# sokunmin/Improved-Body-Parts

Measured on AMD Instinct MI355X. Metric: end-to-end images/sec at 512×512, higher is better.
Workload: dtype f16; 1 GPU; configs[2]+forward: 512x512, flip=on, host->HBM ingest + 4-stage IMHN forward (fp16) + full HIP pafprocess (NMS + limb line-integral + assembly); launch=hipGraph replay, parallelism=image-sharded x1

## Files before the change

improved-body-parts_amd/csrc/posepaf_conv_own.hip:

```cpp
#include <hip/hip_fp16.h>
#include <hip/hip_runtime.h>

#include <atomic>
#include <cstdint>
#include <cstdlib>
#include <type_traits>

#include "../../include/posepaf.h"

namespace {

typedef _Float16 half8_t __attribute__((ext_vector_type(8)));
typedef _Float16 half4_t __attribute__((ext_vector_type(4)));
typedef float float4_t __attribute__((ext_vector_type(4)));

constexpr int BM = 256;
constexpr int NTHREADS = 512;
constexpr int SUB = 1024;

struct ConvParams {
    const _Float16 *x, *w, *bias, *extra, *extra2;
    _Float16 *y, *y2;
    const void *zero;
    int N, H, W, C, K, R, pad, dil, Ho, Wo;
// ... 319 lines not shown
        for (int i = 0; i < PT; i++) xf[i] = *reinterpret_cast<const half8_t *>(sa + (wm * PT + i) * SUB + fragoff);
        const int inflight = np - 1 - ph < 3 ? np - 1 - ph : 3;
        if (inflight == 3) wait_vmcnt<2 * NL>();
        else if (inflight == 2) wait_vmcnt<NL>();
        else if (inflight == 1) wait_vmcnt<0>();
        asm volatile("s_waitcnt lgkmcnt(0)" ::: "memory");
        __builtin_amdgcn_s_barrier();
        __builtin_amdgcn_s_setprio(1);
#pragma unroll
        for (int i = 0; i < PT; i++)
#pragma unroll
            for (int j = 0; j < CT; j++) acc[i][j] = __builtin_amdgcn_mfma_f32_16x16x32_f16(wf[j], xf[i], acc[i][j], 0, 0, 0);
        __builtin_amdgcn_s_setprio(0);
        __builtin_amdgcn_s_barrier();
    }
    if (grp == 0) __builtin_amdgcn_s_barrier();

    epilogue_store<PT, CT>(acc, p, lane, n0 + wn * 64, [&](int i) -> long {
        const long m = m0 + wm * PM + i * 16 + (lane & 15);
        if (m >= p.M) return -1;
        if (!p.up_out) return m;
        const int n = (int)(m / HoWo), rem = (int)(m - (long)n * HoWo);
        const int oy_ = rem / p.Wo, ox_ = rem - oy_ * p.Wo;
        return ((long)n * (2 * p.Ho) + 2 * oy_ + p.py) * (2 * p.Wo) + 2 * ox_ + p.px;
    }, true);
}

constexpr int TP = 512;
constexpr int HALO_RES_SUMS = 2048;
constexpr int HALO_DBG_BITS = HALO_RES_SUMS - 1;

struct HaloParams {
    int TW, TH, lgTW;
    int tiles_x, tiles;
    int HWp, nhalo, npieces;
    int gimg, hrows;
    int tps;
};

__device__ unsigned long long g_conv_clk[8 * 512];

template <int BN, int MASK, int LGTW, int PH = -1, int D = 1>
__global__ __launch_bounds__(NTHREADS) void k_conv3x3_halo(const ConvParams p, const HaloParams hp) {
    constexpr int NT = PH < 0 ? 9 : 4;
    static_assert(D == 1 || PH < 0, "the collapsed upsample form has no dilation");
    constexpr int TW = 1 << LGTW, HWp = TW + 2 * D, TH = TP / TW;
    constexpr int dbg = MASK & HALO_DBG_BITS;
    constexpr int WN = BN / 64;
    constexpr int WM = 8 / WN;
    constexpr int PM = TP / WM;
    constexpr int PT = PM / 16;
    constexpr int CT = 4;
    constexpr int WB = BN * 32 * 2;
    constexpr int KEEP = 3;
    constexpr int NW = 6;
    constexpr int AHEAD = NW - 1;
    constexpr int HP = 56;
#ifdef PP_HALO_NPW7
    constexpr int NPW = 7;
#else
    constexpr int NPW = (LGTW == 7 || D > 1) ? 7 : 6;
#endif
    static_assert(BN == 128, "one weight sub-tile per wave and phase");
    extern __shared__ __align__(16) unsigned char smem[];
    constexpr int halo_bytes = HP * SUB;
    unsigned char *s_halo = smem;
    unsigned char *s_w = smem + 2 * halo_bytes;

    const int lane = threadIdx.x & 63;
    const int wave = __builtin_amdgcn_readfirstlane(threadIdx.x >> 6);
    const int wm = wave / WN, wn = wave % WN;
    const int nct = (p.K + BN - 1) / BN;
    const int ptiles = (p.N / hp.gimg) * hp.tiles, per_xcd = (ptiles + 7) >> 3;
    const int total_ids = 8 * per_xcd * nct;
    const char *wb = reinterpret_cast<const char *>(p.w);
    int n_img = 0, ty0 = 0, tx0 = 0, n0 = 0, t_idx = 0;
    const char *xb = nullptr;
    int hsrc[7];
    const bool p4 = __builtin_amdgcn_readfirstlane(32 + wave < hp.npieces);
    const bool p5 = __builtin_amdgcn_readfirstlane(40 + wave < hp.npieces);
    const bool p6 = __builtin_amdgcn_readfirstlane(48 + wave < hp.npieces);
    unsigned woff = 0;
    int bx_lo = 0, bx_hi = 0, bw_lo = 0, bw_hi = 0, nx = 0, bw_n = 0;
    auto rsrc_of = [&](int lo, int hi, int nbytes) {
        void *base = reinterpret_cast<void *>(((unsigned long long)(unsigned)hi << 32) | (unsigned)lo);
        return __builtin_amdgcn_make_buffer_rsrc(base, 0, nbytes, 0x00020000);
    };
    auto decode = [&](int id) -> bool {
        const int xcd = id & 7, q = id >> 3;
        const int ptile = xcd * per_xcd + q / nct, ctile = q - (q / nct) * nct;
        if (q / nct >= per_xcd || ptile >= ptiles) return false;
        n_img = (ptile / hp.tiles) * hp.gimg;
        const int tile = ptile - (ptile / hp.tiles) * hp.tiles;
        t_idx = tile;
        if (D == 1) ty0 = (tile / hp.tiles_x) * TH;
        else {
            const int trow_ = tile / hp.tiles_x, cls = trow_ / hp.tps;
            ty0 = cls + (trow_ - cls * hp.tps) * TH * D;
        }
        tx0 = (tile - (tile / hp.tiles_x) * hp.tiles_x) * TW;
        n0 = ctile * BN;
        const int sw_ = p.up ? p.W >> 1 : p.W;
        const int ldx = p.ldx ? p.ldx : p.C;
        xb = reinterpret_cast<const char *>(p.x) + (long)n_img * (p.up ? p.H >> 1 : p.H) * sw_ * ldx * 2;
        int ln = lane;
        asm volatile("" : "+v"(ln));
#pragma unroll
        for (int t = 0; t < NPW; t++) {
            const int piece = t * 8 + wave;
            const int phys = piece * SUB + ln * 16;
            const int logical = phys ^ (((phys >> 8) & 1) << 5);
            const int hpix = logical >> 6, chunk = (logical >> 4) & 3;
            const int hy = hpix / HWp, hx = hpix - hy * HWp;
            const int gi = D == 1 ? hy / hp.hrows : 0;
            const int iy = D == 1 ? ty0 - 1 + (hy - gi * hp.hrows) : ty0 + (hy - 1) * D, ix = tx0 - D + hx;
            const bool ok = hpix < hp.nhalo && (unsigned)iy < (unsigned)p.H && (unsigned)ix < (unsigned)p.W;
            hsrc[t] = ok ? (((gi * (p.H >> p.up) + (iy >> p.up)) * sw_ + (ix >> p.up)) * ldx * 2 + chunk * 16)
                         : (int)0x80000000;
        }
        const int b = ln * 16;
        const int bs = b ^ (((b >> 9) & 1) << 5);
        woff = (unsigned)((bs >> 6) * (NT * p.C * 2) + (bs & 63));
        const unsigned long long ax = reinterpret_cast<unsigned long long>(xb);
        const unsigned long long aw = reinterpret_cast<unsigned long long>(wb) + (unsigned long long)((long)(n0 + wave * 16) * ((long)NT * p.C * 2));
        bx_lo = __builtin_amdgcn_readfirstlane((int)(unsigned)ax), bx_hi = __builtin_amdgcn_readfirstlane((int)(unsigned)(ax >> 32));
        bw_lo = __builtin_amdgcn_readfirstlane((int)(unsigned)aw), bw_hi = __builtin_amdgcn_readfirstlane((int)(unsigned)(aw >> 32));
        nx = __builtin_amdgcn_readfirstlane(hp.gimg * (p.up ? p.H >> 1 : p.H) * sw_ * ldx * 2);
        bw_n = __builtin_amdgcn_readfirstlane(n0 + wave * 16 < p.K ? 16 * NT * p.C * 2 : 0);
        return true;
    };
    auto next_tile = [&](int id) -> int {
        while (id < total_ids && !decode(id)) id += gridDim.x;
        return id;
    };

    const int ncb = p.C / 32;
    const int np = ncb * NT;
    int st_cb = 0, st_tap = 0;
    int st_slot = 0;
    int slot_cur = 0;
    auto stage_w = [&]() {
        lds_dma16_buf(rsrc_of(bw_lo, bw_hi, bw_n), woff, (unsigned)((st_tap * p.C + st_cb * 32) * 2), s_w + st_slot * WB + wave * SUB);
        if (++st_slot == NW) st_slot = 0;
        if (++st_tap == NT) {
            st_tap = 0;
            ++st_cb;
        }
    };
    auto stage_halo = [&](int t, int cb, int buf) {
        lds_dma16_buf(rsrc_of(bx_lo, bx_hi, nx), (unsigned)hsrc[t], (unsigned)(cb * 64), s_halo + buf * halo_bytes + (t * 8 + wave) * SUB);
    };

    const int wfrag = (lane & 15) * 64 + (((lane >> 4) * 16) ^ (((lane & 15) >> 3) << 5));
    const int rows_before = (wm * PM) >> LGTW;
    const int hb0 = ((rows_before + (hp.gimg > 1 ? 2 * (rows_before / p.H) : 0)) * HWp + ((wm * PM) & (TW - 1)) + (lane & 15)) * 64 +
                    (lane >> 4) * 16;
    const unsigned lds_halo = (unsigned)(uintptr_t)(__attribute__((address_space(3))) unsigned char *)s_halo;
    const unsigned lds_w = (unsigned)(uintptr_t)(__attribute__((address_space(3))) unsigned char *)s_w + wn * 4 * SUB;
    unsigned R[4][2];
    auto set_R = [&]() {
#pragma unroll
        for (int k = 0; k < 4; k++) {
            const int M = hb0 + k * 64;
            const unsigned a = lds_halo + (unsigned)(M ^ ((M >> 3) & 32));
            R[k][0] = a;
            R[k][1] = a ^ 32u;
        }
    };
    auto flip_R = [&](int to_buf) {
        const unsigned d = to_buf ? (unsigned)halo_bytes : (unsigned)-halo_bytes;
#pragma unroll
        for (int k = 0; k < 4; k++) R[k][0] += d, R[k][1] += d;
    };
    auto xread = [&](auto TAP, auto I, half8_t &dst) {
        constexpr int tap = decltype(TAP)::value, i = decltype(I)::value;
        constexpr int trow = PH < 0 ? tap / 3 : (PH >> 1) + (tap >> 1), tcol = PH < 0 ? D * (tap % 3) : (PH & 1) + (tap & 1);
        constexpr int Cpix = trow * HWp + tcol + ((i * 16) >> LGTW) * HWp + ((i * 16) & (TW - 1));
        constexpr int C = Cpix * 64, k = Cpix & 3, Chi = C & ~255, f = (Chi >> 8) & 1;
        static_assert(Chi < 65536, "16-bit DS offset");
        lds_read16<Chi>(dst, R[k][f]);
    };

    auto stage_first = [&]() {
        st_cb = 0, st_tap = 0, st_slot = 0;
#pragma unroll
        for (int t = 0; t < NPW; t++)
            if (t < 4 || (t == 4 && p4) || (t == 5 && p5) || (t == 6 && p6)) stage_halo(t, 0, 0);
        for (int q = 0; q < AHEAD && q < np; q++) stage_w();
    };
    unsigned long long acc_t[6] = {0, 0, 0, 0, 0, 0}, t_prev = 0;
    auto stamp = [&](int k) {
        if (dbg & 1024) {
            const unsigned long long t = __builtin_amdgcn_s_memtime();
            if (k >= 0) acc_t[k] += t - t_prev;
            t_prev = t;
        }
    };
    int id = next_tile(blockIdx.x);
    if (id >= total_ids) return;
    for (int z = (int)(blockIdx.x >> 3) * p.stagger / (int)((gridDim.x + 7) >> 3); z > 0; z--) __builtin_amdgcn_s_sleep(127);
    stage_first();
  while (true) {
    const int c_img = n_img, c_ty0 = ty0, c_tx0 = tx0, c_n0 = n0, c_tile = t_idx;
    float4_t acc[PT][CT];
#pragma unroll
    for (int i = 0; i < PT; i++)
#pragma unroll
        for (int j = 0; j < CT; j++) acc[i][j] = float4_t{0.f, 0.f, 0.f, 0.f};
    stamp(-1);
    wait_vmcnt<0>();
    __builtin_amdgcn_s_barrier();
    stamp(0);
    slot_cur = 0;
    half8_t wf[CT], xf[PT];
    set_R();
    lds_read16<0>(wf[0], lds_w + wfrag);
    lds_read16<SUB>(wf[1], lds_w + wfrag);
    using T0 = std::integral_constant<int, 0>;
    xread(T0{}, std::integral_constant<int, 0>{}, xf[0]);
    xread(T0{}, std::integral_constant<int, 1>{}, xf[1]);
    xread(T0{}, std::integral_constant<int, 2>{}, xf[2]);
    xread(T0{}, std::integral_constant<int, 3>{}, xf[3]);
    xread(T0{}, std::integral_constant<int, 4>{}, xf[4]);
    xread(T0{}, std::integral_constant<int, 5>{}, xf[5]);
    xread(T0{}, std::integral_constant<int, 6>{}, xf[6]);
    xread(T0{}, std::integral_constant<int, 7>{}, xf[7]);
    wait_lgkmcnt<0>();

    int ph = 0;
    const int grp = wave >> 2;
    unsigned long long rt0 = 0;
    if (dbg & 1024) rt0 = __builtin_amdgcn_s_memrealtime();
    stamp(1);
    auto phase = [&](auto TAP, auto HALO, int cb) {
        constexpr int tap = decltype(TAP)::value;
        constexpr bool halo = decltype(HALO)::value;
        constexpr int ntap = tap == NT - 1 ? 0 : tap + 1;
        constexpr auto halo_at = [](int t) { return t < 0 ? 0 : (NT == 9 ? (t <= 1 ? 2 : (t <= NPW - 3 ? 1 : 0)) : (t == 0 ? NPW : 0)); };
        constexpr int in_flight = KEEP + (!halo ? 0 : NT == 9 ? halo_at(tap) + halo_at(tap - 1) + halo_at(tap - 2) : (tap <= 1 ? NPW : 0));
        static_assert(KEEP == 3, "in_flight sums the halo pieces of three taps");
        auto issue_dma = [&]() {
            if (!(dbg & 1)) {
                if (halo) {
                    if (NT == 4) {
                        if (tap == 0) {
                            stage_halo(0, cb + 1, (cb + 1) & 1);
                            stage_halo(1, cb + 1, (cb + 1) & 1);
                            stage_halo(2, cb + 1, (cb + 1) & 1);
                            stage_halo(3, cb + 1, (cb + 1) & 1);
                            if (p4) stage_halo(4, cb + 1, (cb + 1) & 1);
                            if (p5) stage_halo(5, cb + 1, (cb + 1) & 1);
                            if (NPW == 7 && p6) stage_halo(6, cb + 1, (cb + 1) & 1);
                        }
                    } else if (tap <= 1) {
                        stage_halo(2 * tap, cb + 1, (cb + 1) & 1);
                        stage_halo(2 * tap + 1, cb + 1, (cb + 1) & 1);
                    } else if (tap <= NPW - 3) {
                        if (tap == 2 ? p4 : (tap == 3 ? p5 : p6)) stage_halo(tap + 2, cb + 1, (cb + 1) & 1);
                    }
                }
                if (ph + AHEAD < np) stage_w();
            }
        };
        if (grp == 0 || (dbg & 128)) issue_dma();
        const unsigned sw_cur = lds_w + slot_cur * WB + wfrag;
        if (++slot_cur == NW) slot_cur = 0;
        const unsigned sw_nxt = lds_w + slot_cur * WB + wfrag;
        __builtin_amdgcn_s_setprio(1);
        if (!(dbg & 4)) {
            lds_read16<2 * SUB>(wf[2], sw_cur);
            lds_read16<3 * SUB>(wf[3], sw_cur);
        }
        auto tile_a = [&](auto I) {
            constexpr int i = decltype(I)::value;
            wait_lgkmcnt<9 - i>();
            if (!(dbg & 2)) {
                mfma_acc(acc[i][0], wf[0], xf[i]);
                mfma_acc(acc[i][1], wf[1], xf[i]);
            }
        };
        tile_a(std::integral_constant<int, 0>{});
        tile_a(std::integral_constant<int, 1>{});
        tile_a(std::integral_constant<int, 2>{});
        tile_a(std::integral_constant<int, 3>{});
        tile_a(std::integral_constant<int, 4>{});
        tile_a(std::integral_constant<int, 5>{});
        tile_a(std::integral_constant<int, 6>{});
        tile_a(std::integral_constant<int, 7>{});
        static_assert(PT == 8, "eight pixel tiles per wave");
        constexpr bool refill = !(dbg & 4) && !(tap == NT - 1 && !halo);
        if (grp != 0 && !(dbg & 128)) issue_dma();
        if (refill) {
            lds_read16<0>(wf[0], sw_nxt);
            lds_read16<SUB>(wf[1], sw_nxt);
        }
        wait_lgkmcnt<refill ? 2 : 0>();
        if (refill && tap == NT - 1) flip_R((cb + 1) & 1);
        auto tile_b = [&](auto I) {
            constexpr int i = decltype(I)::value;
            if (!(dbg & 2)) {
                mfma_acc(acc[i][2], wf[2], xf[i]);
                mfma_acc(acc[i][3], wf[3], xf[i]);
            }
            if (refill) xread(std::integral_constant<int, ntap>{}, I, xf[i]);
        };
        tile_b(std::integral_constant<int, 0>{});
        tile_b(std::integral_constant<int, 1>{});
        tile_b(std::integral_constant<int, 2>{});
        tile_b(std::integral_constant<int, 3>{});
        tile_b(std::integral_constant<int, 4>{});
        tile_b(std::integral_constant<int, 5>{});
        tile_b(std::integral_constant<int, 6>{});
        tile_b(std::integral_constant<int, 7>{});
        __builtin_amdgcn_s_setprio(0);
        constexpr bool w4 = halo && (NT == 9 ? (tap >= 2 && tap <= 4) : tap <= 1);
        constexpr bool w5 = halo && (NT == 9 ? (tap >= 3 && tap <= 5) : tap <= 1);
        constexpr bool w6 = halo && NPW == 7 && (NT == 9 ? (tap >= 4 && tap <= 6) : tap <= 1);
        const int missing = (w4 && !p4) + (w5 && !p5) + (w6 && !p6);
        static_assert(in_flight >= 3, "the window always holds the three weight slices");
        if (ph + AHEAD >= np) wait_vmcnt<0>();
        else if (missing == 0) wait_vmcnt<in_flight>();
        else if (missing == 1) wait_vmcnt<(in_flight > 1 ? in_flight - 1 : 0)>();
        else if (missing == 2) wait_vmcnt<(in_flight > 2 ? in_flight - 2 : 0)>();
        else wait_vmcnt<(in_flight > 3 ? in_flight - 3 : 0)>();
        __builtin_amdgcn_s_barrier();
        ++ph;
    };
    auto block = [&](auto HALO, int cb) {
        phase(std::integral_constant<int, 0>{}, HALO, cb);
        phase(std::integral_constant<int, 1>{}, HALO, cb);
        phase(std::integral_constant<int, 2>{}, HALO, cb);
        phase(std::integral_constant<int, 3>{}, HALO, cb);
        if constexpr (NT == 9) {
            phase(std::integral_constant<int, 4>{}, HALO, cb);
            phase(std::integral_constant<int, 5>{}, HALO, cb);
            phase(std::integral_constant<int, 6>{}, HALO, cb);
            phase(std::integral_constant<int, 7>{}, HALO, cb);
            phase(std::integral_constant<int, 8>{}, HALO, cb);
        }
    };
    for (int cb = 0; cb + 1 < ncb; cb++) block(std::true_type{}, cb);
    block(std::false_type{}, ncb - 1);
    asm volatile("s_waitcnt lgkmcnt(0)\n\ts_nop 15\n\ts_nop 15" ::: "memory");
    stamp(2);
    if (dbg & 1024) acc_t[5] += __builtin_amdgcn_s_memrealtime() - rt0;

    id = next_tile(id + gridDim.x);
    const bool has_next = id < total_ids;
    if (has_next) stage_first();
    stamp(3);
    if (dbg & 64)
        epilogue_fullline_probe<PT, CT>(acc, p, lane, c_n0 + wn * 64, [&](int qq) -> long {
            const int q = wm * PM + qq;
            const int qy = q >> LGTW, qx = q & (TW - 1);
            return ((long)c_img * p.H + c_ty0 + qy) * p.W + c_tx0 + qx;
        });
    else if constexpr ((MASK & HALO_RES_SUMS) != 0) {
        if (c_n0 + wn * 64 < p.K)
            epilogue_body<1, PT, CT, true>(acc, p, lane, c_n0 + wn * 64, [&](int i) -> long {
                const int q = wm * PM + i * 16 + (lane & 15);
                return ((long)c_img * p.H + c_ty0 + (q >> LGTW)) * p.W + c_tx0 + (q & (TW - 1));
            }, true, p.csum + ((((long)c_img * hp.tiles + c_tile) * WM) / hp.gimg + wm) * p.K);
    } else
    epilogue_store<PT, CT>(acc, p, lane, c_n0 + wn * 64, [&](int i) -> long {
        const int q = wm * PM + i * 16 + (lane & 15);
        const int qy = q >> LGTW, qx = q & (TW - 1);
        if (PH >= 0)
            return (2 * ((long)c_img * p.H + c_ty0 + qy) + (PH >> 1)) * (2 * p.W) + 2 * (c_tx0 + qx) + (PH & 1);
        if (D > 1) {
            const int ry = c_ty0 + qy * D;
            return ry < p.H ? ((long)c_img * p.H + ry) * p.W + c_tx0 + qx : -1;
        }
        return ((long)c_img * p.H + c_ty0 + qy) * p.W + c_tx0 + qx;
    }, !(dbg & 8), p.csum ? p.csum + (((long)c_img * hp.tiles + c_tile) * WM + wm) * p.K : nullptr);
    stamp(4);
    if (!has_next) break;
  }
    if ((dbg & 1024) && threadIdx.x == 0 && blockIdx.x < 512)
        for (int k = 0; k < 6; k++) g_conv_clk[blockIdx.x * 8 + k] = acc_t[k];
}

constexpr int kMaxDevices = 32, kMaxInst = 192;
struct DevState {
    void *zero = nullptr;
    int ncu = 0;
    bool attr[kMaxInst] = {};
};
DevState g_dev[kMaxDevices];
std::atomic<int> g_inst_count{0};

DevState *dev_state() {
    int dev = 0;
    if (hipGetDevice(&dev) != hipSuccess || dev < 0 || dev >= kMaxDevices) return nullptr;
    return &g_dev[dev];
}
bool capturing(hipStream_t st) {
    hipStreamCaptureStatus cs = hipStreamCaptureStatusNone;
    return hipStreamIsCapturing(st, &cs) == hipSuccess && cs != hipStreamCaptureStatusNone;
}
int ensure_attr(const void *fn, int lds, int inst, hipStream_t st) {
    DevState *d = dev_state();
    if (!d || inst < 0 || inst >= kMaxInst) return PP_ERR_HIP;
    if (d->attr[inst]) return PP_OK;
    if (capturing(st)) return PP_ERR_UNSUPPORTED;
    if (hipFuncSetAttribute(fn, hipFuncAttributeMaxDynamicSharedMemorySize, lds) != hipSuccess) return PP_ERR_HIP;
    d->attr[inst] = true;
    return PP_OK;
}


bool halo_geometry(const ConvParams &p, HaloParams &g) {
    if (p.R != 3 || p.pad != p.dil || p.dil < 1 || p.C % 32 || p.K % 64) return false;
    if (p.dil != 1 && (p.dil < 3 || p.dil > 5 || p.up || p.csum)) return false;
    if ((long)p.H * p.W * (p.ldx ? p.ldx : p.C) * 2 >= (1L << 31)) return false;
    int tw = 128;
    while (tw >= 16 && p.W % tw) tw >>= 1;
    if (tw < 16) return false;
    const int th = TP / tw;
    g.TW = tw;
    g.TH = th;
    g.lgTW = 0;
    while ((1 << g.lgTW) < tw) g.lgTW++;
    g.HWp = tw + 2 * p.dil;
    g.tps = 0;
    if (p.dil > 1) {
        if (tw < 32) return false;
        g.gimg = 1;
        g.hrows = th + 2;
        g.tiles_x = p.W / tw;
        g.tps = ((p.H + p.dil - 1) / p.dil + th - 1) / th;
        g.tiles = g.tiles_x * p.dil * g.tps;
        g.nhalo = (th + 2) * (tw + 2 * p.dil);
// ... 28 lines not shown
    if (!ds) return PP_ERR_HIP;
    if (ds->ncu == 0) {
        int dev = 0, n = 0;
        if (hipGetDevice(&dev) != hipSuccess || hipDeviceGetAttribute(&n, hipDeviceAttributeMultiprocessorCount, dev) != hipSuccess)
            return PP_ERR_HIP;
        ds->ncu = n >= 8 ? (n / 8) * 8 : 8;
    }
    const int ncu = ds->ncu;
    static const bool persist = [] {
        const char *e = getenv("POSEPAF_CONV_PERSIST");
        return !(e && e[0] == '0');
    }();
    const dim3 grid(persist && ids > (unsigned)ncu ? (unsigned)ncu : ids);
    ConvParams q = p;
    if (q.stagger < 0) {
        const float rounds = (float)ids / (float)grid.x;
        const float f = 0.5f * (rounds < 32.f ? rounds / 32.f : 1.f);
        q.stagger = grid.x < ids ? (int)(f * (float)(p.C / 32 * (PH < 0 ? 9 : 4)) * 1500.f / 8128.f + 0.5f) : 0;
    }
    hipLaunchKernelGGL((k_conv3x3_halo<128, MASK, LGTW, PH, D>), grid, dim3(NTHREADS), lds, st, q, g);
    return hipGetLastError() == hipSuccess ? PP_OK : PP_ERR_HIP;
}

template <int D>
int launch_halo_dilated(const ConvParams &p, const HaloParams &g, hipStream_t st) {
    switch (g.lgTW) {
        case 7: return launch_halo_inst<0, 7, -1, D>(p, g, st);
        case 6: return launch_halo_inst<0, 6, -1, D>(p, g, st);
        case 5: return launch_halo_inst<0, 5, -1, D>(p, g, st);
        default: return PP_ERR_UNSUPPORTED;
    }
}

template <int MASK>
int launch_halo_mask(const ConvParams &p, const HaloParams &g, hipStream_t st) {
    if (p.dil != 1) {
        if (MASK != 0) return PP_ERR_UNSUPPORTED;
        return p.dil == 3 ? launch_halo_dilated<3>(p, g, st) : (p.dil == 4 ? launch_halo_dilated<4>(p, g, st) : launch_halo_dilated<5>(p, g, st));
    }
    if (g.lgTW == 7) return launch_halo_inst<MASK, 7>(p, g, st);
    if (MASK == 0) {
        if (g.lgTW == 6) return launch_halo_inst<0, 6>(p, g, st);
        if (g.lgTW == 5) return launch_halo_inst<0, 5>(p, g, st);
        if (g.lgTW == 4) return launch_halo_inst<0, 4>(p, g, st);
    }
    return PP_ERR_UNSUPPORTED;
}

template <int PH>
int launch_halo_phase(const ConvParams &p, const HaloParams &g, hipStream_t st) {
    switch (g.lgTW) {
        case 7: return launch_halo_inst<0, 7, PH>(p, g, st);
        case 6: return launch_halo_inst<0, 6, PH>(p, g, st);
        case 5: return launch_halo_inst<0, 5, PH>(p, g, st);
        case 4: return launch_halo_inst<0, 4, PH>(p, g, st);
        default: return PP_ERR_UNSUPPORTED;
    }
}

int launch_halo_res_sums(const ConvParams &p, const HaloParams &g, hipStream_t st) {
    switch (g.lgTW) {
        case 7: return launch_halo_inst<HALO_RES_SUMS, 7>(p, g, st);
        case 6: return launch_halo_inst<HALO_RES_SUMS, 6>(p, g, st);
        case 5: return launch_halo_inst<HALO_RES_SUMS, 5>(p, g, st);
        case 4: return launch_halo_inst<HALO_RES_SUMS, 4>(p, g, st);
        default: return PP_ERR_UNSUPPORTED;
    }
}

int launch_halo(const ConvParams &p, const HaloParams &g, hipStream_t st) {
    switch (p.dbg) {
        case 0: return launch_halo_mask<0>(p, g, st);
#ifdef PP_CONV_DIAG
        case 1: return launch_halo_mask<1>(p, g, st);
        case 4: return launch_halo_mask<4>(p, g, st);
        case 6: return launch_halo_mask<6>(p, g, st);
        case 5: return launch_halo_mask<5>(p, g, st);
        case 7: return launch_halo_mask<7>(p, g, st);
        case 15: return launch_halo_mask<15>(p, g, st);
        case 64: return launch_halo_mask<64>(p, g, st);
        case 71: return launch_halo_mask<71>(p, g, st);
        case 1152: return launch_halo_mask<1152>(p, g, st);
        case 1024: return launch_halo_mask<1024>(p, g, st);
        case 1028: return launch_halo_mask<1028>(p, g, st);
        case 1029: return launch_halo_mask<1029>(p, g, st);
#endif
        default: return PP_ERR_BAD_ARG;
    }
}

template <int BN>
int launch(const ConvParams &p, hipStream_t st) {
    constexpr int lds = 4 * (BM * 32 * 2 + BN * 32 * 2);
    static const int inst = g_inst_count.fetch_add(1);
    if (const int rc = ensure_attr(reinterpret_cast<const void *>(&k_conv_igemm<BN>), lds, inst, st)) return rc;
    const dim3 grid((unsigned)((p.M + BM - 1) / BM), (unsigned)(p.K / BN));
    hipLaunchKernelGGL(k_conv_igemm<BN>, grid, dim3(NTHREADS), lds, st, p);
    return hipGetLastError() == hipSuccess ? PP_OK : PP_ERR_HIP;
}


struct PwParams {
    const _Float16 *x, *scale, *w;
    ConvParams e;
    long M;
    int Kin, hw, n_per_wg;
    const _Float16 *x2;
    int kt1;
    _Float16 *pool;
    int W;
    const _Float16 *pre_add = nullptr;
};

template <int KT, int PT, int EX, bool POOL, bool PRE = false>
__global__ __launch_bounds__(512) void k_pw(const PwParams p) {
    extern __shared__ __align__(16) unsigned char smem[];
    const int lane = threadIdx.x & 63;
    const int wave = __builtin_amdgcn_readfirstlane(threadIdx.x >> 6);
    const int n_base = blockIdx.y * p.n_per_wg;
    const int Nw = p.e.K - n_base < p.n_per_wg ? p.e.K - n_base : p.n_per_wg;
    constexpr int KG = KT * 4;
    for (int i = threadIdx.x; i < Nw * KG; i += 512) {
        const int n = i / KG, q = i - n * KG;
        const int t = q >> 2, g = q & 3, r16 = n & 15, nt = n >> 4;
        const half8_t v = *reinterpret_cast<const half8_t *>(p.w + (long)(n_base + n) * (KT * 32) + q * 8);
        *reinterpret_cast<half8_t *>(smem + (nt * KT + t) * SUB + r16 * 64 + ((g * 16) ^ ((r16 >> 3) << 5))) = v;
    }
    __syncthreads();
    const int wfrag = (lane & 15) * 64 + (((lane >> 4) * 16) ^ (((lane & 15) >> 3) << 5));
    const int g = lane >> 4, pl = lane & 15;
    constexpr int GP = PT * 16;
    constexpr int CB = PT >= 2 ? PT / 2 : 1;
    constexpr bool pooling = POOL;
    const long groups = (p.M + GP - 1) / GP;
    const int cblocks = pooling ? p.W / (16 * CB) : 1;
    for (long grp = (long)blockIdx.x * 8 + wave; grp < groups; grp += (long)gridDim.x * 8) {
        const long rp = pooling ? grp / cblocks : 0;
        const int cbk = pooling ? (int)(grp - rp * cblocks) : 0;
        auto tile_m = [&](int i) -> long {
            return pooling ? (2 * rp + i / CB) * p.W + (long)(cbk * CB + i % CB) * 16 : grp * GP + 16 * i;
        };
        const long m0 = tile_m(0);
        half8_t xf[PT][KT];
#pragma unroll
        for (int i = 0; i < PT; i++) {
            const long m = tile_m(i) + pl;
            const long mm = m < p.M ? m : 0;
            const _Float16 *row = p.x + mm * (p.kt1 * 32) + g * 8;
            const _Float16 *row2 = p.x2 ? p.x2 + mm * ((KT - p.kt1) * 32) + g * 8 - p.kt1 * 32 : row;
#pragma unroll
            for (int t = 0; t < KT; t++) xf[i][t] = *reinterpret_cast<const half8_t *>((t < p.kt1 ? row : row2) + t * 32);
        }
        if (p.scale) {
            const _Float16 *sc = p.scale + (m0 / p.hw) * (KT * 32) + g * 8;
#pragma unroll
            for (int t = 0; t < KT; t++) {
                const half8_t sv = *reinterpret_cast<const half8_t *>(sc + t * 32);
#pragma unroll
                for (int i = 0; i < PT; i++) xf[i][t] = xf[i][t] * sv;
            }
        }
        if constexpr (PRE) {
            if (p.pre_add) {
#pragma unroll
                for (int i = 0; i < PT; i++) {
                    const long m = tile_m(i) + pl;
// ... 402 lines not shown
        HaloParams g;
        if (halo_geometry(p, g)) return launch_halo(p, g, st);
        if (bn != 0 || ldx != c_in || ldy != c_out) return PP_ERR_UNSUPPORTED;
        bn = c_out % 256 == 0 ? 256 : (c_out % 128 == 0 ? 128 : 64);
    }
    switch (bn) {
        case 256: return launch<256>(p, st);
        case 128: return launch<128>(p, st);
        default: return launch<64>(p, st);
    }
}

PP_API int pp_conv_own_sums_splits(int h, int wd) {
    ConvParams q;
    q.R = 3, q.pad = 1, q.dil = 1, q.C = 32, q.K = 128, q.H = h, q.W = wd, q.N = 1, q.csum = nullptr;
    HaloParams g;
    return (halo_geometry(q, g) && g.gimg == 1) ? g.tiles * 4 : 0;
}
PP_API int pp_conv_own_sums_f16(const void *x, const void *w, const void *bias, void *y, void *sums_ws, int n, int h, int wd, int c_in,
                                int c_out, float slope, void *stream) {
    if (!x || !w || !bias || !y || !sums_ws || n <= 0 || h <= 0 || wd <= 0) return PP_ERR_BAD_ARG;
    if (!pp_conv_own_supported(c_in, c_out, 3) || !(slope >= 0.f && slope <= 1.f)) return PP_ERR_UNSUPPORTED;
    if ((reinterpret_cast<uintptr_t>(x) | reinterpret_cast<uintptr_t>(w) | reinterpret_cast<uintptr_t>(bias) | reinterpret_cast<uintptr_t>(y) |
         reinterpret_cast<uintptr_t>(sums_ws)) & 15)
        return PP_ERR_BAD_ARG;
    hipStream_t st = static_cast<hipStream_t>(stream);
    ConvParams p;
    p.x = static_cast<const _Float16 *>(x), p.w = static_cast<const _Float16 *>(w), p.bias = static_cast<const _Float16 *>(bias);
    p.extra = nullptr, p.extra2 = nullptr, p.up = 0, p.y = static_cast<_Float16 *>(y), p.y2 = nullptr, p.zero = nullptr;
    p.N = n, p.H = h, p.W = wd, p.C = c_in, p.K = c_out, p.R = 3, p.pad = 1, p.dil = 1, p.Ho = h, p.Wo = wd;
    p.ldy = c_out, p.csum = static_cast<float *>(sums_ws), p.M = (long)n * h * wd, p.mode = 0, p.slope = slope, p.dbg = 0, p.stagger = -1;
    p.pad_y = p.pad_x = 1, p.up_out = 0, p.py = p.px = 0;
    HaloParams g;
    if (!halo_geometry(p, g)) return PP_ERR_UNSUPPORTED;
    return launch_halo(p, g, st);
}

PP_API int pp_conv_own_res_sums_splits(int h, int wd) {
    ConvParams q;
    q.R = 3, q.pad = 1, q.dil = 1, q.C = 32, q.K = 128, q.H = h, q.W = wd, q.N = 32, q.csum = nullptr, q.up = 0, q.ldx = 0, q.mode = 1;
    HaloParams g;
    return halo_geometry(q, g) ? g.tiles * 4 / g.gimg : 0;
}
PP_API int pp_conv_own_res_sums_f16(const void *x, const void *w, const void *bias, const void *residual, void *y, void *sums_ws, int n,
                                    int h, int wd, int c_in, int c_out, float slope, void *stream) {
    if (!x || !w || !bias || !residual || !y || !sums_ws || n <= 0 || h <= 0 || wd <= 0) return PP_ERR_BAD_ARG;
    if (!pp_conv_own_supported(c_in, c_out, 3) || !(slope >= 0.f && slope <= 1.f)) return PP_ERR_UNSUPPORTED;
    if ((reinterpret_cast<uintptr_t>(x) | reinterpret_cast<uintptr_t>(w) | reinterpret_cast<uintptr_t>(bias) | reinterpret_cast<uintptr_t>(y) |
         reinterpret_cast<uintptr_t>(residual) | reinterpret_cast<uintptr_t>(sums_ws)) & 15)
        return PP_ERR_BAD_ARG;
    hipStream_t st = static_cast<hipStream_t>(stream);
    ConvParams p;
    p.x = static_cast<const _Float16 *>(x), p.w = static_cast<const _Float16 *>(w), p.bias = static_cast<const _Float16 *>(bias);
    p.extra = static_cast<const _Float16 *>(residual), p.extra2 = nullptr, p.up = 0, p.y = static_cast<_Float16 *>(y), p.y2 = nullptr, p.zero = nullptr;
    p.N = n, p.H = h, p.W = wd, p.C = c_in, p.K = c_out, p.R = 3, p.pad = 1, p.dil = 1, p.Ho = h, p.Wo = wd;
    p.ldy = c_out, p.csum = static_cast<float *>(sums_ws), p.M = (long)n * h * wd, p.mode = 1, p.slope = slope, p.dbg = 0, p.stagger = -1;
    p.pad_y = p.pad_x = 1, p.up_out = 0, p.py = p.px = 0;
    HaloParams g;
    if (!halo_geometry(p, g)) return PP_ERR_UNSUPPORTED;
    return launch_halo_res_sums(p, g, st);
}

PP_API int pp_conv_up2_collapsed_f16(const void *x, const void *w4, const void *bias, const void *extra, const void *extra2, void *y, int n,
                                     int h_low, int w_low, int c_in, int c_out, int extra_mode, float slope, int bn, void *stream) {
    if (!x || !w4 || !bias || !y || n <= 0 || h_low <= 0 || w_low <= 0 || (extra_mode != 0 && extra_mode != 2 && extra_mode != 3) ||
        (extra_mode != 0) != (extra != nullptr) || (extra_mode == 3) != (extra2 != nullptr))
        return PP_ERR_BAD_ARG;
    if (!pp_conv_own_supported(c_in, c_out, 2) || !(slope >= 0.f && slope <= 1.f)) return PP_ERR_UNSUPPORTED;
    if ((reinterpret_cast<uintptr_t>(x) | reinterpret_cast<uintptr_t>(w4) | reinterpret_cast<uintptr_t>(bias) | reinterpret_cast<uintptr_t>(extra) |
         reinterpret_cast<uintptr_t>(extra2) | reinterpret_cast<uintptr_t>(y)) & 15)
        return PP_ERR_BAD_ARG;
    hipStream_t st = static_cast<hipStream_t>(stream);
    if (bn == 512) {
        ConvParams q;
        q.x = static_cast<const _Float16 *>(x), q.bias = static_cast<const _Float16 *>(bias);
        q.extra = static_cast<const _Float16 *>(extra), q.extra2 = static_cast<const _Float16 *>(extra2);
        q.y = static_cast<_Float16 *>(y), q.y2 = nullptr, q.zero = nullptr, q.up = 0;
        q.N = n, q.H = h_low, q.W = w_low, q.C = c_in, q.K = c_out, q.R = 3, q.pad = 1, q.dil = 1, q.Ho = h_low, q.Wo = w_low;
        q.ldy = c_out, q.csum = nullptr, q.M = (long)n * h_low * w_low, q.mode = extra_mode, q.slope = slope, q.dbg = 0, q.stagger = -1;
        q.pad_y = q.pad_x = 1, q.up_out = 1, q.py = q.px = 0;
        HaloParams g;
        if (!halo_geometry(q, g)) return PP_ERR_UNSUPPORTED;
        const long wphase = (long)c_out * 4 * c_in;
        for (int ph = 0; ph < 4; ph++) {
            q.w = static_cast<const _Float16 *>(w4) + ph * wphase;
            const int rc = ph == 0 ? launch_halo_phase<0>(q, g, st) : (ph == 1 ? launch_halo_phase<1>(q, g, st) :
                           (ph == 2 ? launch_halo_phase<2>(q, g, st) : launch_halo_phase<3>(q, g, st)));
            if (rc != PP_OK) return rc;
        }
        return PP_OK;
    }
    if (bn == 0) bn = c_out % 256 == 0 ? 256 : (c_out % 128 == 0 ? 128 : 64);
    if ((bn != 256 && bn != 128 && bn != 64) || c_out % bn) return PP_ERR_UNSUPPORTED;
    DevState *ds = dev_state();
    if (!ds) return PP_ERR_HIP;
    if (!ds->zero) {
        if (capturing(st)) return PP_ERR_UNSUPPORTED;
        if (hipMalloc(&ds->zero, 256) != hipSuccess || hipMemset(ds->zero, 0, 256) != hipSuccess) return PP_ERR_HIP;
    }
    ConvParams p;
    p.x = static_cast<const _Float16 *>(x), p.bias = static_cast<const _Float16 *>(bias);
    p.extra = static_cast<const _Float16 *>(extra), p.extra2 = static_cast<const _Float16 *>(extra2);
    p.y = static_cast<_Float16 *>(y), p.y2 = nullptr, p.zero = ds->zero, p.up = 0;
    p.N = n, p.H = h_low, p.W = w_low, p.C = c_in, p.K = c_out, p.R = 2, p.pad = 0, p.dil = 1, p.Ho = h_low, p.Wo = w_low;
    p.ldy = c_out, p.csum = nullptr, p.M = (long)n * h_low * w_low, p.mode = extra_mode, p.slope = slope, p.dbg = 0, p.stagger = -1;
    p.up_out = 1;
    const long wphase = (long)c_out * 4 * c_in;
    for (int ph = 0; ph < 4; ph++) {
        p.py = ph >> 1, p.px = ph & 1;
        p.pad_y = 1 - p.py, p.pad_x = 1 - p.px;
        p.w = static_cast<const _Float16 *>(w4) + ph * wphase;
        const int rc = bn == 256 ? launch<256>(p, st) : (bn == 128 ? launch<128>(p, st) : launch<64>(p, st));
        if (rc != PP_OK) return rc;
    }
    return PP_OK;
}

PP_API int pp_conv_own_f16(const void *x, const void *w, const void *bias, const void *extra, void *y, int n, int h, int wd, int c_in,
                    int c_out, int ksize, int pad, int dilation, int extra_mode, float slope, int bn, void *stream) {
    if (extra_mode > 2) return PP_ERR_BAD_ARG;
    return pp_conv_own_ex_f16(x, w, bias, extra, nullptr, y, nullptr, n, h, wd, c_in, c_out, ksize, pad, dilation, extra_mode, slope, bn, 0,
                              stream);
}

}
```

Baseline: 978.8 images/sec.

## Stream next tile's halo and weight loads during last channel block of persistent conv

In the persistent halo implicit-GEMM conv kernel, the next tile is now decoded early and its first halo pieces and weight slices are prefetched while the current tile's last channel block is still computing. Previously the pipeline drained and the next tile's first stage was issued serially. The per-lane halo geometry is precomputed once into packed registers so that per-tile decoding is cheaper. Halo buffer parity is now tracked explicitly. This hides the tile-transition latency at the cost of extra register pressure and more complex wait-count logic.

Result: no change. 983.5 images/sec, median of 6 (+0.5%).

```diff
diff --git a/improved-body-parts_amd/csrc/posepaf_conv_own.hip b/improved-body-parts_amd/csrc/posepaf_conv_own.hip
--- a/improved-body-parts_amd/csrc/posepaf_conv_own.hip
+++ b/improved-body-parts_amd/csrc/posepaf_conv_own.hip
@@ -425,11 +425,12 @@
     const bool p6 = __builtin_amdgcn_readfirstlane(48 + wave < hp.npieces);
     unsigned woff = 0;
     int bx_lo = 0, bx_hi = 0, bw_lo = 0, bw_hi = 0, nx = 0, bw_n = 0;
+    int nbw_lo = 0, nbw_hi = 0, nbw_n = 0;
     auto rsrc_of = [&](int lo, int hi, int nbytes) {
         void *base = reinterpret_cast<void *>(((unsigned long long)(unsigned)hi << 32) | (unsigned)lo);
         return __builtin_amdgcn_make_buffer_rsrc(base, 0, nbytes, 0x00020000);
     };
-    auto decode = [&](int id) -> bool {
+    auto decode_tile = [&](int id) __attribute__((always_inline)) -> bool {
         const int xcd = id & 7, q = id >> 3;
         const int ptile = xcd * per_xcd + q / nct, ctile = q - (q / nct) * nct;
         if (q / nct >= per_xcd || ptile >= ptiles) return false;
@@ -446,34 +447,43 @@
         const int sw_ = p.up ? p.W >> 1 : p.W;
         const int ldx = p.ldx ? p.ldx : p.C;
         xb = reinterpret_cast<const char *>(p.x) + (long)n_img * (p.up ? p.H >> 1 : p.H) * sw_ * ldx * 2;
-        int ln = lane;
-        asm volatile("" : "+v"(ln));
-#pragma unroll
-        for (int t = 0; t < NPW; t++) {
-            const int piece = t * 8 + wave;
-            const int phys = piece * SUB + ln * 16;
-            const int logical = phys ^ (((phys >> 8) & 1) << 5);
-            const int hpix = logical >> 6, chunk = (logical >> 4) & 3;
-            const int hy = hpix / HWp, hx = hpix - hy * HWp;
-            const int gi = D == 1 ? hy / hp.hrows : 0;
-            const int iy = D == 1 ? ty0 - 1 + (hy - gi * hp.hrows) : ty0 + (hy - 1) * D, ix = tx0 - D + hx;
-            const bool ok = hpix < hp.nhalo && (unsigned)iy < (unsigned)p.H && (unsigned)ix < (unsigned)p.W;
-            hsrc[t] = ok ? (((gi * (p.H >> p.up) + (iy >> p.up)) * sw_ + (ix >> p.up)) * ldx * 2 + chunk * 16)
-                         : (int)0x80000000;
-        }
-        const int b = ln * 16;
-        const int bs = b ^ (((b >> 9) & 1) << 5);
-        woff = (unsigned)((bs >> 6) * (NT * p.C * 2) + (bs & 63));
         const unsigned long long ax = reinterpret_cast<unsigned long long>(xb);
         const unsigned long long aw = reinterpret_cast<unsigned long long>(wb) + (unsigned long long)((long)(n0 + wave * 16) * ((long)NT * p.C * 2));
         bx_lo = __builtin_amdgcn_readfirstlane((int)(unsigned)ax), bx_hi = __builtin_amdgcn_readfirstlane((int)(unsigned)(ax >> 32));
-        bw_lo = __builtin_amdgcn_readfirstlane((int)(unsigned)aw), bw_hi = __builtin_amdgcn_readfirstlane((int)(unsigned)(aw >> 32));
+        nbw_lo = __builtin_amdgcn_readfirstlane((int)(unsigned)aw), nbw_hi = __builtin_amdgcn_readfirstlane((int)(unsigned)(aw >> 32));
         nx = __builtin_amdgcn_readfirstlane(hp.gimg * (p.up ? p.H >> 1 : p.H) * sw_ * ldx * 2);
-        bw_n = __builtin_amdgcn_readfirstlane(n0 + wave * 16 < p.K ? 16 * NT * p.C * 2 : 0);
+        nbw_n = __builtin_amdgcn_readfirstlane(n0 + wave * 16 < p.K ? 16 * NT * p.C * 2 : 0);
         return true;
     };
-    auto next_tile = [&](int id) -> int {
-        while (id < total_ids && !decode(id)) id += gridDim.x;
+    int hgeo[7];
+#pragma unroll
+    for (int t = 0; t < NPW; t++) {
+        const int phys = (t * 8 + wave) * SUB + lane * 16;
+        const int logical = phys ^ (((phys >> 8) & 1) << 5);
+        const int hpix = logical >> 6, chunk = (logical >> 4) & 3;
+        const int hy = hpix / HWp, hx = hpix - hy * HWp;
+        const int gi = D == 1 ? hy / hp.hrows : 0;
+        hgeo[t] = hx | ((D == 1 ? hy - gi * hp.hrows : hy) & 255) << 8 | (gi & 255) << 16 | chunk << 24 | (hpix < hp.nhalo ? 1 << 26 : 0);
+    }
+    static_assert(HWp <= 255 && TH + 2 <= 255, "hgeo's fields");
+    auto decode_piece = [&](int t) __attribute__((always_inline)) {
+        const int sw_ = p.up ? p.W >> 1 : p.W;
+        const int ldx = p.ldx ? p.ldx : p.C;
+        int g = hgeo[t];
+        asm volatile("" : "+v"(g));
+        const int hx = g & 255, r = (g >> 8) & 255, gi = (g >> 16) & 255, chunk = (g >> 24) & 3;
+        const int iy = D == 1 ? ty0 - 1 + r : ty0 + (r - 1) * D, ix = tx0 - D + hx;
+        const bool ok = (g >> 26) && (unsigned)iy < (unsigned)p.H && (unsigned)ix < (unsigned)p.W;
+        hsrc[t] = ok ? (((gi * (p.H >> p.up) + (iy >> p.up)) * sw_ + (ix >> p.up)) * ldx * 2 + chunk * 16)
+                     : (int)0x80000000;
+    };
+    {
+        const int b = lane * 16;
+        const int bs = b ^ (((b >> 9) & 1) << 5);
+        woff = (unsigned)((bs >> 6) * (NT * p.C * 2) + (bs & 63));
+    }
+    auto next_tile = [&](int id) __attribute__((always_inline)) -> int {
+        while (id < total_ids && !decode_tile(id)) id += gridDim.x;
         return id;
     };
 
@@ -482,15 +492,17 @@
     int st_cb = 0, st_tap = 0;
     int st_slot = 0;
     int slot_cur = 0;
-    auto stage_w = [&]() {
+    int cur_buf = 0;
+    bool stream = false;
+    auto stage_w = [&]() __attribute__((always_inline)) {
         lds_dma16_buf(rsrc_of(bw_lo, bw_hi, bw_n), woff, (unsigned)((st_tap * p.C + st_cb * 32) * 2), s_w + st_slot * WB + wave * SUB);
         if (++st_slot == NW) st_slot = 0;
         if (++st_tap == NT) {
             st_tap = 0;
-            ++st_cb;
+            if (++st_cb == ncb) st_cb = 0, bw_lo = nbw_lo, bw_hi = nbw_hi, bw_n = nbw_n;
         }
     };
-    auto stage_halo = [&](int t, int cb, int buf) {
+    auto stage_halo = [&](int t, int cb, int buf) __attribute__((always_inline)) {
         lds_dma16_buf(rsrc_of(bx_lo, bx_hi, nx), (unsigned)hsrc[t], (unsigned)(cb * 64), s_halo + buf * halo_bytes + (t * 8 + wave) * SUB);
     };
 
@@ -505,7 +517,7 @@
 #pragma unroll
         for (int k = 0; k < 4; k++) {
             const int M = hb0 + k * 64;
-            const unsigned a = lds_halo + (unsigned)(M ^ ((M >> 3) & 32));
+            const unsigned a = lds_halo + (cur_buf ? (unsigned)halo_bytes : 0u) + (unsigned)(M ^ ((M >> 3) & 32));
             R[k][0] = a;
             R[k][1] = a ^ 32u;
         }
@@ -524,13 +536,17 @@
         lds_read16<Chi>(dst, R[k][f]);
     };
 
-    auto stage_first = [&]() {
-        st_cb = 0, st_tap = 0, st_slot = 0;
-#pragma unroll
-        for (int t = 0; t < NPW; t++)
+    auto stage_first = [&]() __attribute__((always_inline)) {
+        st_cb = 0, st_tap = 0, st_slot = 0, slot_cur = 0, cur_buf = 0;
+        bw_lo = nbw_lo, bw_hi = nbw_hi, bw_n = nbw_n;
+#pragma unroll
+        for (int t = 0; t < NPW; t++) {
+            decode_piece(t);
             if (t < 4 || (t == 4 && p4) || (t == 5 && p5) || (t == 6 && p6)) stage_halo(t, 0, 0);
+        }
         for (int q = 0; q < AHEAD && q < np; q++) stage_w();
     };
+    const bool can_stream = !(dbg & (1 | 256)) && (NT == 9 || ncb >= 2);
     unsigned long long acc_t[6] = {0, 0, 0, 0, 0, 0}, t_prev = 0;
     auto stamp = [&](int k) {
         if (dbg & 1024) {
@@ -554,11 +570,11 @@
     wait_vmcnt<0>();
     __builtin_amdgcn_s_barrier();
     stamp(0);
-    slot_cur = 0;
+    stream = false;
     half8_t wf[CT], xf[PT];
     set_R();
-    lds_read16<0>(wf[0], lds_w + wfrag);
-    lds_read16<SUB>(wf[1], lds_w + wfrag);
+    lds_read16<0>(wf[0], lds_w + slot_cur * WB + wfrag);
+    lds_read16<SUB>(wf[1], lds_w + slot_cur * WB + wfrag);
     using T0 = std::integral_constant<int, 0>;
     xread(T0{}, std::integral_constant<int, 0>{}, xf[0]);
     xread(T0{}, std::integral_constant<int, 1>{}, xf[1]);
@@ -575,34 +591,39 @@
     unsigned long long rt0 = 0;
     if (dbg & 1024) rt0 = __builtin_amdgcn_s_memrealtime();
     stamp(1);
-    auto phase = [&](auto TAP, auto HALO, int cb) {
+    auto phase = [&](auto TAP, auto LAST, int cb) {
         constexpr int tap = decltype(TAP)::value;
-        constexpr bool halo = decltype(HALO)::value;
+        constexpr bool last = decltype(LAST)::value;
         constexpr int ntap = tap == NT - 1 ? 0 : tap + 1;
         constexpr auto halo_at = [](int t) { return t < 0 ? 0 : (NT == 9 ? (t <= 1 ? 2 : (t <= NPW - 3 ? 1 : 0)) : (t == 0 ? NPW : 0)); };
-        constexpr int in_flight = KEEP + (!halo ? 0 : NT == 9 ? halo_at(tap) + halo_at(tap - 1) + halo_at(tap - 2) : (tap <= 1 ? NPW : 0));
+        constexpr int halo_in_flight = NT == 9 ? halo_at(tap) + halo_at(tap - 1) + halo_at(tap - 2) : (tap <= 1 ? NPW : 0);
         static_assert(KEEP == 3, "in_flight sums the halo pieces of three taps");
+        const bool halo = !last || stream;
+        auto piece = [&](int t) __attribute__((always_inline)) {
+            if (last) decode_piece(t);
+            stage_halo(t, last ? 0 : cb + 1, cur_buf ^ 1);
+        };
         auto issue_dma = [&]() {
             if (!(dbg & 1)) {
                 if (halo) {
                     if (NT == 4) {
                         if (tap == 0) {
-                            stage_halo(0, cb + 1, (cb + 1) & 1);
-                            stage_halo(1, cb + 1, (cb + 1) & 1);
-                            stage_halo(2, cb + 1, (cb + 1) & 1);
-                            stage_halo(3, cb + 1, (cb + 1) & 1);
-                            if (p4) stage_halo(4, cb + 1, (cb + 1) & 1);
-                            if (p5) stage_halo(5, cb + 1, (cb + 1) & 1);
-                            if (NPW == 7 && p6) stage_halo(6, cb + 1, (cb + 1) & 1);
+                            piece(0);
+                            piece(1);
+                            piece(2);
+                            piece(3);
+                            if (p4) piece(4);
+                            if (p5) piece(5);
+                            if (NPW == 7 && p6) piece(6);
                         }
                     } else if (tap <= 1) {
-                        stage_halo(2 * tap, cb + 1, (cb + 1) & 1);
-                        stage_halo(2 * tap + 1, cb + 1, (cb + 1) & 1);
+                        piece(2 * tap);
+                        piece(2 * tap + 1);
                     } else if (tap <= NPW - 3) {
-                        if (tap == 2 ? p4 : (tap == 3 ? p5 : p6)) stage_halo(tap + 2, cb + 1, (cb + 1) & 1);
+                        if (tap == 2 ? p4 : (tap == 3 ? p5 : p6)) piece(tap + 2);
                     }
                 }
-                if (ph + AHEAD < np) stage_w();
+                if (ph + AHEAD < np || stream) stage_w();
             }
         };
         if (grp == 0 || (dbg & 128)) issue_dma();
@@ -631,14 +652,14 @@
         tile_a(std::integral_constant<int, 6>{});
         tile_a(std::integral_constant<int, 7>{});
         static_assert(PT == 8, "eight pixel tiles per wave");
-        constexpr bool refill = !(dbg & 4) && !(tap == NT - 1 && !halo);
+        constexpr bool refill = !(dbg & 4) && !(tap == NT - 1 && last);
         if (grp != 0 && !(dbg & 128)) issue_dma();
         if (refill) {
             lds_read16<0>(wf[0], sw_nxt);
             lds_read16<SUB>(wf[1], sw_nxt);
         }
         wait_lgkmcnt<refill ? 2 : 0>();
-        if (refill && tap == NT - 1) flip_R((cb + 1) & 1);
+        if (refill && tap == NT - 1) flip_R(cur_buf ^ 1);
         auto tile_b = [&](auto I) {
             constexpr int i = decltype(I)::value;
             if (!(dbg & 2)) {
@@ -656,12 +677,13 @@
         tile_b(std::integral_constant<int, 6>{});
         tile_b(std::integral_constant<int, 7>{});
         __builtin_amdgcn_s_setprio(0);
-        constexpr bool w4 = halo && (NT == 9 ? (tap >= 2 && tap <= 4) : tap <= 1);
-        constexpr bool w5 = halo && (NT == 9 ? (tap >= 3 && tap <= 5) : tap <= 1);
-        constexpr bool w6 = halo && NPW == 7 && (NT == 9 ? (tap >= 4 && tap <= 6) : tap <= 1);
+        constexpr bool w4 = NT == 9 ? (tap >= 2 && tap <= 4) : tap <= 1;
+        constexpr bool w5 = NT == 9 ? (tap >= 3 && tap <= 5) : tap <= 1;
+        constexpr bool w6 = NPW == 7 && (NT == 9 ? (tap >= 4 && tap <= 6) : tap <= 1);
         const int missing = (w4 && !p4) + (w5 && !p5) + (w6 && !p6);
-        static_assert(in_flight >= 3, "the window always holds the three weight slices");
-        if (ph + AHEAD >= np) wait_vmcnt<0>();
+        constexpr int in_flight = KEEP + halo_in_flight;
+        if (ph + AHEAD >= np && !stream) wait_vmcnt<0>();
+        else if (!halo) wait_vmcnt<KEEP>();
         else if (missing == 0) wait_vmcnt<in_flight>();
         else if (missing == 1) wait_vmcnt<(in_flight > 1 ? in_flight - 1 : 0)>();
         else if (missing == 2) wait_vmcnt<(in_flight > 2 ? in_flight - 2 : 0)>();
@@ -669,8 +691,14 @@
         __builtin_amdgcn_s_barrier();
         ++ph;
     };
+    auto advance = [&]() __attribute__((always_inline)) {
+        id = next_tile(id + gridDim.x);
+        stream = id < total_ids;
+    };
     auto block = [&](auto HALO, int cb) {
         phase(std::integral_constant<int, 0>{}, HALO, cb);
+        if constexpr (NT == 4 && !decltype(HALO)::value)
+            if (can_stream && cb == ncb - 2) advance();
         phase(std::integral_constant<int, 1>{}, HALO, cb);
         phase(std::integral_constant<int, 2>{}, HALO, cb);
         phase(std::integral_constant<int, 3>{}, HALO, cb);
@@ -682,15 +710,22 @@
             phase(std::integral_constant<int, 8>{}, HALO, cb);
         }
     };
-    for (int cb = 0; cb + 1 < ncb; cb++) block(std::true_type{}, cb);
-    block(std::false_type{}, ncb - 1);
+    for (int cb = 0; cb + 1 < ncb; cb++) {
+        block(std::false_type{}, cb);
+        cur_buf ^= 1;
+    }
+    if (NT == 9 && can_stream) advance();
+    block(std::true_type{}, ncb - 1);
+    cur_buf ^= 1;
     asm volatile("s_waitcnt lgkmcnt(0)\n\ts_nop 15\n\ts_nop 15" ::: "memory");
     stamp(2);
     if (dbg & 1024) acc_t[5] += __builtin_amdgcn_s_memrealtime() - rt0;
 
-    id = next_tile(id + gridDim.x);
-    const bool has_next = id < total_ids;
-    if (has_next) stage_first();
+    if (!can_stream) {
+        advance();
+        if (stream) stage_first();
+    }
+    const bool has_next = stream;
     stamp(3);
     if (dbg & 64)
         epilogue_fullline_probe<PT, CT>(acc, p, lane, c_n0 + wn * 64, [&](int qq) -> long {
@@ -885,6 +920,7 @@
         case 71: return launch_halo_mask<71>(p, g, st);
         case 1152: return launch_halo_mask<1152>(p, g, st);
         case 1024: return launch_halo_mask<1024>(p, g, st);
+        case 1280: return launch_halo_mask<1280>(p, g, st);
         case 1028: return launch_halo_mask<1028>(p, g, st);
         case 1029: return launch_halo_mask<1029>(p, g, st);
 #endif
@@ -1453,8 +1489,18 @@
         HaloParams g;
         if (!halo_geometry(q, g)) return PP_ERR_UNSUPPORTED;
         const long wphase = (long)c_out * 4 * c_in;
+#ifdef PP_CONV_DIAG
+        static const int dbg = std::getenv("POSEPAF_CONV_DBG") ? std::atoi(std::getenv("POSEPAF_CONV_DBG")) : 0;
+#else
+        const int dbg = 0;
+#endif
         for (int ph = 0; ph < 4; ph++) {
             q.w = static_cast<const _Float16 *>(w4) + ph * wphase;
+#ifdef PP_CONV_DIAG
+            if (ph == 3 && g.lgTW == 6 && (dbg == 1024 || dbg == 1280))
+                return dbg == 1024 ? launch_halo_inst<1024, 6, 3>(q, g, st) : launch_halo_inst<1280, 6, 3>(q, g, st);
+#endif
+            (void)dbg;
             const int rc = ph == 0 ? launch_halo_phase<0>(q, g, st) : (ph == 1 ? launch_halo_phase<1>(q, g, st) :
                            (ph == 2 ? launch_halo_phase<2>(q, g, st) : launch_halo_phase<3>(q, g, st)));
             if (rc != PP_OK) return rc;
```
